# risc-mi/totalsegmentator2D

Measured on AMD Instinct MI355X. Metric: 2-ch 512x512 slices/sec, higher is better.
Workload: dtype f32 storage/accumulate, products as 3x fp16-split MFMA (f16x3)

## Files before the change

totalsegmentator2d_amd/csrc/dispatch.cpp:

```cpp
#include "engine_internal.h"
#include "tile_dims.h"

#include <algorithm>

namespace ts2d {

namespace {

inline int lg_exact(int v) { return (v > 0 && (v & (v - 1)) == 0) ? ilog2(v) : -1; }

inline void tile_finish(TileGeom& g, int B, int Ht, int Wt, int sy, int sx, int taps) {
    const bool p2 = lg_exact(g.TH) >= 0 && lg_exact(g.TW) >= 0;
    g.lgTH = p2 ? ilog2(g.TH) : -1; g.lgTW = p2 ? ilog2(g.TW) : -1;
    if (g.NIMG > 1) { g.tiles_x = 1; g.tiles_y = 1; }
    else { g.tiles_x = (Wt + g.TW - 1) / g.TW; g.tiles_y = (Ht + g.TH - 1) / g.TH; }
    g.n_mtiles = (B + g.NIMG - 1) / g.NIMG * g.tiles_x * g.tiles_y;
    const int halo = (taps == 9) ? 3 : 1;
    g.PH = (g.TH - 1) * sy + halo; g.PW = (g.TW - 1) * sx + halo;
}

TileGeom tile_geom_pow2(int B, int Ht, int Wt, int sy, int sx, int taps) {
    TileGeom g{};
    g.TW = std::min(32, pow2ceil(Wt));
    g.TH = std::min(pow2ceil(Ht), kBM / g.TW);
// ... 65 lines not shown
            if (th * tw > best || (th * tw == best && tw > g.TW)) { best = th * tw; g.TH = th; g.TW = tw; }
        }
    }
    if (best < 192) return g;
    ok = true;
    g.NIMG = 1;
    tile_finish(g, B, Ht, Wt, 2, 2, 9);
    return g;
}

TileGeom tile_fixed(int B, int Ht, int Wt, int th, int tw, int sy, int sx) {
    TileGeom g{};
    g.TH = th; g.TW = tw; g.NIMG = 1;
    tile_finish(g, B, Ht, Wt, sy, sx, 9);
    return g;
}
int choose_ksplit(const Op& op, const TileGeom& g) {
    if (op.type != OP_CONV || !op.split_ok || op.first_direct) return 1;
    if (g.NIMG < 4) return 1;
    const int nchunks = (op.cin + op.cin_skip) / (op.stride == 1 ? 16 : 8);
    int S = 1;
    while (S < 8 && nchunks / (S * 2) >= 4) S *= 2;
    return S;
}

int fill_ksplit(const ts2d_engine* e, long long n_wgs, int nchunks, bool full) {
    if (!e->use_sbk || full || e->num_cus > 256) return 1;
    int S = 1;
    while (S < 8 && n_wgs * S < e->num_cus && nchunks / (S * 2) >= 4) S *= 2;
    return S;
}

inline bool fits32(size_t bytes) { return bytes < ((size_t)1 << 31); }
inline bool magic_ok(const TileGeom& g) { return (unsigned long long)g.n_mtiles * (unsigned)(g.tiles_x * g.tiles_y) < 0x100000000ull; }

constexpr int kUpqMin = 256;
constexpr int kH2Min = 64;

int segment_tiles(const ts2d_engine* e, const TileGeom& g) {
    const int tpi = g.tiles_x * g.tiles_y, want = std::min(g.n_mtiles, 2 * e->num_cus);
    int seg = 1;
    for (int d = 1; d <= tpi; ++d) if (tpi % d == 0 && g.n_mtiles / d >= want) seg = d;
    return seg;
}

bool fuse0_applies(const ts2d_engine* e, int H, int W) {
// ... 122 lines not shown
    if (op.stride == 2) {
        int s2k = 1;
        {
            const TileGeom g1 = tile_geom(B, Ht, Wt, 2, 2, 9);
            const int P1 = g1.PH * g1.PW * g1.NIMG;
            if (e->use_one && g1.NIMG == 1 && P1 <= 5 * kBlock && img32) s2k = fill_ksplit(e, (long long)g1.n_mtiles * (op.cout / c.bn), op.cin / 8, full);
        }
        if (s2k == 1 && op.s2v2_ok && e->use_s2v2 && e->use_one && Ht % 8 == 0 && Wt % 32 == 0 && img32 && magic_ok(tile_fixed(B, Ht, Wt, 8, 32, 2, 2))) {
            c.k = K_S2_V2; c.bn = op.bn2; c.fused_stats = true;
            c.g = tile_fixed(B, Ht, Wt, 8, 32, 2, 2);
            s2v2_variant(e, op, c);
            return c;
        }
        if (s2k == 1 && op.s2v2_ok && e->use_s2v2 && e->use_one && e->use_flex2 && img32 && (f16 || e->use_flex2 > 1)) {
            bool ok = false;
            const TileGeom gs = tile_geom_s2v2(B, Ht, Wt, ok);
            if (ok && magic_ok(gs)) { c.k = K_S2_V2; c.bn = op.bn2; c.fused_stats = true; c.flex = true; c.g = gs; s2v2_variant(e, op, c); return c; }
        }
        c.g = tile_geom(B, Ht, Wt, 2, 2, 9);
        c.ksplit = std::max(choose_ksplit(op, c.g), s2k);
        c.fused_stats = c.g.NIMG == 1 && c.ksplit == 1;
        const int P = c.g.PH * c.g.PW * c.g.NIMG;
        c.k = (e->use_one && c.g.NIMG == 1 && P <= 5 * kBlock && img32) ? K_S2_ONE : K_S2_GENERIC;
        return c;
    }
    if (op.res_ok && e->use_res && e->use_one && src.normed && op.skip < 0 && Ht % 8 == 0 && Wt % 32 == 0 && fits32((size_t)Ht * Wt * 32 * 4)) {
        c.k = (oi == 1 && fuse0_applies(e, H, W)) ? K_S1_RES32F : K_S1_RES32;
        c.fused_stats = true;
        c.g = tile_fixed(B, Ht, Wt, 8, 32, 1, 1);
        c.seg = segment_tiles(e, c.g);
        return c;
    }
    c.g = tile_geom(B, Ht, Wt, 1, 1, 9);
    c.ksplit = choose_ksplit(op, c.g);
    c.fused_stats = c.g.NIMG == 1;
    const int P = c.g.PH * c.g.PW * c.g.NIMG;
    const bool srcs_normed = src.normed && (op.skip < 0 || e->tensors[op.skip].normed);
    const bool tiles16 = Ht % 16 == 0 && Wt % 32 == 0 && c.g.NIMG == 1 && img32;
    if (c.g.NIMG == 1 && img32 && op.cout % c.bn == 0) {
        const bool can = f16 ? (op.h32_ok && P * 4 <= 6 * kBlock) : (e->use_one && P * 2 <= 3 * kBlock);
        const int sk = can ? fill_ksplit(e, (long long)c.g.n_mtiles * (op.cout / c.bn), ct / (f16 ? 32 : 16), full) : 1;
        if (sk > 1) {
            c.ksplit = sk; c.fused_stats = false;
            c.k = f16 ? K_S1_H32 : K_S1_ONE;
            return c;
        }
    }
    if (f16) {
        if (e->use_h2 && tiles16 && op.cout % 64 == 0 && op.skip < 0 && ct % 32 == 0 && src.normed && ct >= kH2Min) {
            c.k = K_S1_H2; c.bn = 64;
            c.g = tile_fixed(B, Ht, Wt, 16, 32, 1, 1);
            return c;
        }
        c.k = (op.h32_ok && c.g.NIMG == 1 && P * 4 <= 6 * kBlock && img32) ? K_S1_H32 : K_S1_GENERIC;
        return c;
    }
    const bool one = e->use_one && c.g.NIMG == 1 && P * 2 <= 3 * kBlock && img32;
    if (one && e->use_q && tiles16 && c.bn == 64 && ct >= 64 && srcs_normed && magic_ok(tile_fixed(B, Ht, Wt, 16, 32, 1, 1))) {
        c.k = K_S1_QP;
        c.g = tile_fixed(B, Ht, Wt, 16, 32, 1, 1);
        return c;
    }
    c.k = one ? K_S1_ONE : K_S1_GENERIC;
    return c;
}

const char* kernel_name(const Op& op, const Choice& c) {
    const bool b64 = c.bn == 64;
    switch (c.k) {
    case K_NONE: case K_FUSED_AWAY: return "";
    case K_FIRST: return c.first_split ? "conv3x3_first_split" : "conv3x3_first";
    case K_FIRST_STATS: return "conv3x3_first_stats";
    case K_EXACT: return op.type == OP_CONV ? "conv_mfma_f32" : "convT_mfma_f32";
    case K_S1_GENERIC: return "conv3x3_f16x3";
    case K_S1_ONE: return b64 ? "conv3x3_f16x3_one<64>" : "conv3x3_f16x3_one<32>";
    case K_S1_QP: return "conv3x3_f16x3_qp";
    case K_S1_H32: return b64 ? "conv3x3_h32<64>" : "conv3x3_h32<32>";
    case K_S1_H2: return "conv3x3_h2";
    case K_S1_RES32: return "conv3x3_res32";
    case K_S1_RES32F: return "conv3x3_res32f";
    case K_S2_V2: return c.bn == 128 ? (c.k32 ? "conv3x3s2_v2<128,k32>" : "conv3x3s2_v2<128>") : (c.k32 ? "conv3x3s2_v2<64,k32>" : "conv3x3s2_v2<64>");
    case K_S2_ONE: return "conv3x3s2_f16x3_one";
    case K_S2_GENERIC: return "conv3x3s2_f16x3";
    case K_T_ONE: case K_T_GENERIC: return "convT2x2_f16x3";
    case K_UP0: return "conv3x3_up0";
    case K_UPQ: return "conv3x3_upq";
// ... 154 lines not shown
```

totalsegmentator2d_amd/csrc/engine.hip:

```cpp
#include "engine_internal.h"
#include "kernels.h"
#include "kernels_f16x3.h"
#include "kernels_f16x3_convt.h"
#include "kernels_h32.h"
#include "kernels_head.h"
#include "kernels_f16x3_one.h"
#include "kernels_f16x3_qp.h"
#include "kernels_first.h"
#include "kernels_res32.h"
#include "kernels_s2v2.h"
#include "kernels_s2v2p.h"
#include "kernels_upc.h"
#include "kernels_up0.h"
#include "kernels_upq.h"
#include "kernels_upc_h.h"
#include "kernels_upc_h2.h"
#include "kernels_resblock.h"

#include <atomic>
#include <cstdio>
#include <cmath>
#include <cstdlib>
#include <cstring>
#include <string>
// ... 339 lines not shown
    return TS2D_OK;
}

template <int TAPS, int SY, int SX, int CK, int EPI, typename ST = float>
hipError_t launch_exact_bn(bool b64, const ConvArgs& a, dim3 grid, size_t smem, hipStream_t st) {
    return b64 ? launch_max_lds<conv_mfma_f32<TAPS, SY, SX, CK, 64, EPI, ST>>(grid, dim3(kBlock), smem, st, a)
               : launch_max_lds<conv_mfma_f32<TAPS, SY, SX, CK, 32, EPI, ST>>(grid, dim3(kBlock), smem, st, a);
}
hipError_t launch_exact(int taps, int sy, int sx, int ck, int bn, bool f16, const ConvArgs& a, dim3 grid, size_t smem, hipStream_t st) {
    const bool b64 = bn == 64;
    if (bn != 32 && bn != 64) return hipErrorInvalidConfiguration;
    if (taps == 9 && sy == 1 && sx == 1 && !f16) {
        if (ck == 16) return launch_exact_bn<9, 1, 1, 16, 0>(b64, a, grid, smem, st);
        if (ck == 8) return launch_exact_bn<9, 1, 1, 8, 0>(b64, a, grid, smem, st);
    }
    if (taps == 9 && sy == 2 && sx == 2 && ck == 8 && !f16) return launch_exact_bn<9, 2, 2, 8, 0>(b64, a, grid, smem, st);
    if (taps == 9 && sy == 2 && sx == 1 && ck == 8) return f16 ? launch_exact_bn<9, 2, 1, 8, 0, _Float16>(b64, a, grid, smem, st) : launch_exact_bn<9, 2, 1, 8, 0>(b64, a, grid, smem, st);
    if (taps == 9 && sy == 1 && sx == 2 && ck == 8) return f16 ? launch_exact_bn<9, 1, 2, 8, 0, _Float16>(b64, a, grid, smem, st) : launch_exact_bn<9, 1, 2, 8, 0>(b64, a, grid, smem, st);
    if (taps == 1 && ck == 16)
        return f16 ? launch_exact_bn<1, 1, 1, 16, 1, _Float16>(b64, a, grid, smem, st) : launch_exact_bn<1, 1, 1, 16, 1>(b64, a, grid, smem, st);
    return hipErrorInvalidConfiguration;
}

hipError_t launch_tiled(Kern k, bool f16, int bn, int P, const ConvArgs& a, int grid_x, size_t smem, hipStream_t st) {
    const dim3 grid(grid_x, a.ksplit), block(kBlock);
    const bool b64 = bn == 64;
    if (bn != 32 && bn != 64) return hipErrorInvalidConfiguration;
    switch (k) {
    case K_S1_ONE:
        return b64 ? launch_max_lds<conv3x3_f16x3_one<64, true>>(grid, block, smem, st, a) : launch_max_lds<conv3x3_f16x3_one<32, false>>(grid, block, smem, st, a);
    case K_S1_H32:
        return b64 ? launch_max_lds<conv3x3_h32<64, 6>>(grid, block, smem, st, a) : launch_max_lds<conv3x3_h32<32, 6>>(grid, block, smem, st, a);
    default: break;
    }
    return with_storage(f16, [&](auto s) {
        using S = decltype(s); using ST = typename S::type;
        if (k == K_S2_ONE)
            return b64 ? launch_max_lds<conv3x3s2_f16x3_one<64, false, false, ST, S::np>>(grid, block, smem, st, a)
                       : launch_max_lds<conv3x3s2_f16x3_one<32, false, false, ST, S::np>>(grid, block, smem, st, a);
        if (k == K_S1_GENERIC) {
            if (P * 2 <= 3 * kBlock)
                return b64 ? launch_max_lds<conv3x3_f16x3<64, 3, 1, ST, S::np>>(grid, block, smem, st, a) : launch_max_lds<conv3x3_f16x3<32, 3, 1, ST, S::np>>(grid, block, smem, st, a);
            return b64 ? launch_max_lds<conv3x3_f16x3<64, 5, 1, ST, S::np>>(grid, block, smem, st, a) : launch_max_lds<conv3x3_f16x3<32, 5, 1, ST, S::np>>(grid, block, smem, st, a);
        }
        if (k == K_S2_GENERIC) {
            if (P <= 5 * kBlock)
                return b64 ? launch_max_lds<conv3x3s2_f16x3<64, 5, ST, S::np>>(grid, block, smem, st, a) : launch_max_lds<conv3x3s2_f16x3<32, 5, ST, S::np>>(grid, block, smem, st, a);
            return b64 ? launch_max_lds<conv3x3s2_f16x3<64, 6, ST, S::np>>(grid, block, smem, st, a) : launch_max_lds<conv3x3s2_f16x3<32, 6, ST, S::np>>(grid, block, smem, st, a);
        }
        return hipErrorInvalidConfiguration;
    });
}

hipError_t launch_s2v2(const ts2d_engine* e, const Choice& c, bool f16, const ConvArgs& ca, int grid_x, hipStream_t st) {
    const size_t wchunk = s2v2_wchunk(c);
    const bool resw = s2v2_resident(c);
    const dim3 grid(std::min(grid_x, 8 * ca.n_ctiles * std::max(1, e->num_cus / (8 * ca.n_ctiles)))), block(kS2Threads);
    const size_t smem = (size_t)c.npp * 2 * kS2Plane + (resw ? (size_t)c.nch : 1) * wchunk;
    if (c.s2p) return launch_max_lds<conv3x3s2_v2p>(grid, block, kS2pLds, st, ca);
    auto inst = [&](auto bn_, auto s, auto k32_) {
        using S = decltype(s); using ST = typename S::type;
        constexpr int BN = decltype(bn_)::value; constexpr bool K32 = decltype(k32_)::value;
// ... 65 lines not shown
    case K_S1_QP: {
        ca.wph = wts + op.dev_wp; ca.oscale = wts + op.dev_ws;
        const int gridp = std::min(grid, 8 * ca.n_ctiles * std::max(1, e->num_cus / (8 * ca.n_ctiles)));
        le = launch_max_lds<conv3x3_f16x3_qp>(dim3(gridp), dim3(kQThreads), kQpLds, r.st, ca);
        break;
    }
    default: {
        const bool s2 = op.stride == 2;
        size_t smem = std::max((size_t)(((P * (op.ck + 4) + 3) & ~3) + taps * (op.ck / 8) * bn * 8) * sizeof(float),
                               (size_t)4 * bn * 4 * sizeof(float));
        if (c.k != K_EXACT) {
            smem = !s2 ? (size_t)P * kRec + (size_t)9 * bn * kRec : (size_t)P * kRec8 + (size_t)5 * bn * kRec;
            smem = std::max(smem, (size_t)4 * bn * 4 * sizeof(float));
            ca.wph = wts + (c.k == K_S1_H32 ? op.dev_wh32 : op.dev_wh); ca.oscale = wts + op.dev_ws;
        }
        if (c.ksplit > 1) {
            ca.ksplit = c.ksplit; ca.kslice_stride = (long long)r.B * Ht * Wt * op.cout;
            ca.dst = e->d_partial; ca.part = nullptr;
        }
        if (smem > 160 * 1024) return fail(TS2D_ERR_INVALID, "op %s: LDS tile of %zu bytes exceeds 160 KiB", op.name.c_str(), smem);
        if (c.k == K_EXACT) {
            const bool aniso = conv ? op.stride == 3 : op.stride != 2;
            le = launch_exact(taps, conv ? op.sy : 1, conv ? op.sx : 1, op.ck, bn, r.f16 && aniso, ca, dim3(grid), smem, r.st);
        } else le = launch_tiled(c.k, r.f16, bn, P, ca, grid, smem, r.st);
        break;
    }
    }
    if (le != hipSuccess) return hip_failed(op, le);
    return TS2D_OK;
}

int launch_stats(ts2d_engine* e, size_t oi, const Choice& c, const Run& r) {
    const Op& op = e->ops[oi];
    Tensor& dst = e->tensors[op.dst];
    const float* wts = e->d_weights;
    const float *bias = wts + op.dev_b, *gamma = wts + op.dev_g, *beta = wts + op.dev_be;
    const float eps = e->arch.norm_eps;
    const int B = r.B, C = op.cout, HW = (r.H >> op.ly) * (r.W >> op.lx);
    const hipStream_t st = r.st;
    const dim3 per_image(B, C / 32);
    int ntiles = 0;
    TRY(prof_begin(e, op.name, ".stats", st)); prof_kernel(e, "finalize_stats");
    with_storage(r.f16, [&](auto s) {
        using ST = typename decltype(s)::type;
        ST* out = reinterpret_cast<ST*>(dst.data);
        const long long stride = (long long)B * HW * C;
        if (c.ksplit > 1 && HW == 256)
// ... 191 lines not shown

int ts2d_engine_weight_buffer(ts2d_engine* e, void** dev_ptr, size_t* n_bytes) {
    if (!e || !dev_ptr || !n_bytes) return fail(TS2D_ERR_INVALID, "ts2d_engine_weight_buffer: null argument");
    *dev_ptr = e->d_weights; *n_bytes = e->weight_floats * sizeof(float);
    return TS2D_OK;
}

int ts2d_engine_set_precision(ts2d_engine* e, int mode) {
    if (!e) return fail(TS2D_ERR_INVALID, "ts2d_engine_set_precision: null engine");
    if (mode != TS2D_PRECISION_F32_EXACT && mode != TS2D_PRECISION_F32_SPLIT_F16X3 && mode != TS2D_PRECISION_F16)
        return fail(TS2D_ERR_INVALID, "unknown precision mode %d", mode);
    if (mode == TS2D_PRECISION_F16 && e->residual && !e->use_resf16)
        return fail(TS2D_ERR_INVALID, "TS2D_PRECISION_F16 is not supported on a residual-encoder engine (TS2D_PRECISION_F32_SPLIT_F16X3 and "
                    "TS2D_PRECISION_F32_EXACT are); the mode is unchanged");
    e->precision = mode;
    return TS2D_OK;
}

int ts2d_engine_set_option(ts2d_engine* e, const char* name, int value) {
    if (!e || !name) return fail(TS2D_ERR_INVALID, "ts2d_engine_set_option: null argument");
    struct B { const char* n; bool* p; };
    struct I { const char* n; int* p; int lo, hi; };
    const B bools[] = {{"one", &e->use_one}, {"s2v2", &e->use_s2v2}, {"q", &e->use_q}, {"h2", &e->use_h2},  {"uh2", &e->use_uh2},
                       {"first_split", &e->use_first_split}, {"sbk", &e->use_sbk}, {"s2k32", &e->use_s2k32}, {"s2p", &e->use_s2p}, {"up0", &e->use_up0}, {"upc", &e->use_upc}, {"res", &e->use_res}, {"fuse0", &e->use_fuse0}, {"flex", &e->use_flex}, {"resf16", &e->use_resf16}};
    const I ints[] = {{"u0seg", &e->u0seg, 0, 1 << 20}, {"flex2", &e->use_flex2, 0, 2}};
    bool found = false;
    for (const B& b : bools) if (!strcmp(name, b.n)) { *b.p = value != 0; found = true; }
    for (const I& i : ints) if (!strcmp(name, i.n)) {
        if (value < i.lo || value > i.hi) return fail(TS2D_ERR_INVALID, "option %s = %d out of range [%d, %d]", name, value, i.lo, i.hi);
        *i.p = value; found = true;
    }
    if (!found) return fail(TS2D_ERR_INVALID, "unknown option '%s' (one s2v2 q h2 uh2 up0 u0seg upc res fuse0 flex flex2 first_split sbk s2k32 s2p resf16)", name);
    e->ws_precision = -1;
    ++e->opt_gen;
    return TS2D_OK;
}

int ts2d_engine_set_keep_activations(ts2d_engine* e, int enable) {
    if (!e) return fail(TS2D_ERR_INVALID, "ts2d_engine_set_keep_activations: null engine");
    e->keep_activations = enable != 0;
    return TS2D_OK;
}

int ts2d_engine_set_tile_dtype(ts2d_engine* e, int mode) {
    if (!e) return fail(TS2D_ERR_INVALID, "ts2d_engine_set_tile_dtype: null engine");
    if (mode != TS2D_TILE_F32 && mode != TS2D_TILE_F16) return fail(TS2D_ERR_INVALID, "unknown tile dtype %d", mode);
    e->tile_half = mode == TS2D_TILE_F16;
    return TS2D_OK;
}

int ts2d_engine_weights_ready(ts2d_engine* e) {
    if (!e) return fail(TS2D_ERR_INVALID, "ts2d_engine_weights_ready: null engine");
    e->weights_ready = true;
    return TS2D_OK;
}
// ... 243 lines not shown
```

totalsegmentator2d_amd/csrc/engine_internal.h:

```cpp
#pragma once
#include "../../include/ts2d_engine.h"
#include <hip/hip_runtime_api.h>
#include "device_tables.h"
#include "tile_dims.h"

#include <atomic>
#include <cstddef>
#include <cstdint>
#include <string>
#include <vector>

#pragma GCC visibility push(hidden)
namespace ts2d {

int fail(int code, const char* fmt, ...) __attribute__((format(printf, 2, 3)));
const char* last_error();

#define HIP_TRY(expr)                                                                                     \
    do {                                                                                                  \
        hipError_t _e = (expr);                                                                           \
        if (_e != hipSuccess)                                                                             \
            return fail(_e == hipErrorOutOfMemory ? TS2D_ERR_NOMEM : TS2D_ERR_HIP, "%s failed: %s (%s:%d)", \
                        #expr, hipGetErrorString(_e), __FILE__, __LINE__);                                \
    } while (0)
// ... 68 lines not shown

struct Launch { std::string name, kernel; int ksplit = 1; hipEvent_t e0 = nullptr, e1 = nullptr; };

inline size_t align_up(size_t v, size_t a) { return (v + a - 1) / a * a; }

struct TileGeom { int TH, TW, NIMG, lgTH, lgTW, tiles_x, tiles_y, n_mtiles, PH, PW; };

enum Kern { K_NONE = 0, K_FUSED_AWAY, K_FIRST, K_FIRST_STATS, K_EXACT, K_S1_GENERIC, K_S1_ONE, K_S1_QP, K_S1_H32, K_S1_H2, K_S1_RES32, K_S1_RES32F,
            K_S2_V2, K_S2_ONE, K_S2_GENERIC, K_T_ONE, K_T_GENERIC, K_UP0, K_UPQ, K_UPC, K_UPC_H, K_UPC_H2, K_HEAD_MFMA, K_HEAD_1X1, K_PROJ, K_JOIN };

struct Choice {
    Kern k = K_NONE;
    TileGeom g{};
    int bn = 0;
    int ksplit = 1;
    bool fused_stats = false;
    int ppt = 1;
    bool first_full = false;
    bool flex = false;
    bool first_split = false;
    bool k32 = false;
    int npp = 0, nch = 0;
    bool s2p = false;
    int seg = 0;
    int ks = 0;
    bool half = false;
    const char* name = "";
};

inline int pow2ceil(int v) { int p = 1; while (p < v) p <<= 1; return p; }
inline int ilog2(int v) { int l = 0; while ((1 << l) < v) ++l; return l; }
inline int ct_total(const Op& op) { return op.cin + op.cin_skip; }
inline size_t s2v2_wchunk(const Choice& c) { return (size_t)9 * c.npp * 2 * c.bn * 16; }
inline bool s2v2_resident(const Choice& c) { return (size_t)c.npp * 2 * kS2PlaneBytes + (size_t)c.nch * s2v2_wchunk(c) <= (size_t)kS2LdsMax; }

}

#pragma GCC visibility pop

struct ts2d_engine {
    ts2d_arch_desc arch{};
    int lvl_y[TS2D_MAX_STAGES] = {0}, lvl_x[TS2D_MAX_STAGES] = {0};
    int device = 0;
    int cin_pad = 8;
    std::vector<ts2d::Tensor> tensors;
    std::vector<ts2d::Op> ops;
    size_t blob_floats = 0;
    ts2d_arch_desc user_arch{};
    bool residual = false;
    int n_blocks[TS2D_MAX_STAGES] = {0};
    bool padded = false;
    size_t user_blob_floats = 0;
    float* d_weights = nullptr; size_t weight_floats = 0;
    bool weights_ready = false;
    int precision = TS2D_PRECISION_F32_SPLIT_F16X3;
    int num_cus = 256;
    int tile_half = 0;
    int tiled_inf = 0;
    bool use_one = true;
    bool use_s2v2 = true;
    bool use_q = true;
    bool use_h2 = true;
    bool use_uh2 = true;
    bool use_s2k32 = true;
    bool use_s2p = true;
    bool use_sbk = true;
    bool use_first_split = true;
    bool use_up0 = true;
    int u0seg = 0;
    bool use_upc = true;
    bool use_res = true;
    bool use_fuse0 = true;
    bool diagnosing = false;
    int use_flex2 = 2;
    bool use_resf16 = false;
    bool use_flex = true;
    int dbg = 0;
    unsigned long long* d_prof = nullptr;
    std::vector<char> fused_away;
    char* d_ws = nullptr; size_t ws_bytes = 0; int wsB = 0, wsH = 0, wsW = 0;
    bool ws_external = false;
    uint32_t ws_token = 0;
    std::vector<ts2d::Choice> plan; int planB = 0, planH = 0, planW = 0, plan_prec = -1; unsigned plan_gen = 0, opt_gen = 1; bool plan_full = false;
    char* d_stage = nullptr; size_t stage_bytes = 0;
    bool ws_full = false;
    bool last_full = false;
    int ws_precision = -1; bool ws_keep = false;
    bool keep_activations = false;
// ... 81 lines not shown
```

totalsegmentator2d_amd/csrc/kernels_f16x3.h:

```cpp
#pragma once
#include "kernels.h"

typedef _Float16 half8 __attribute__((ext_vector_type(8)));

namespace ts2d {

constexpr int kRec = 80;

template <typename ST> struct Raw8;
template <> struct Raw8<float> {
    f32x4 a, b;
    __device__ __forceinline__ void zero() { a = f32x4{0.f, 0.f, 0.f, 0.f}; b = a; }
    __device__ __forceinline__ void load(const void* base, size_t off) {
        const float* p = reinterpret_cast<const float*>(base) + off;
        a = *reinterpret_cast<const f32x4*>(p); b = *reinterpret_cast<const f32x4*>(p + 4);
    }
    __device__ __forceinline__ void get(f32x4& va, f32x4& vb) const { va = a; vb = b; }
};
template <> struct Raw8<_Float16> {
    half8 h;
    __device__ __forceinline__ void zero() {
#pragma unroll
        for (int e = 0; e < 8; ++e) h[e] = (_Float16)0.f;
    }
// ... 179 lines not shown
                const unsigned soff = (unsigned)((((rowoff & (TW - 1)) + (rowoff >> a.lgTW) * a.Wt) * a.Cout) * (int)sizeof(ST));
                float v = __builtin_fmaf(acc_t[mt][nt][i], oscale, bv);
                buffer_store_act<ST>(v, rs, voff, soff);
                const float d = round_act<ST>(v) - kv;
                s += d; q = __builtin_fmaf(d, d, q);
            }
        }
        st_s[nt] = s; st_q[nt] = q; st_k[nt] = kv;
    }
    if (a.part != nullptr) {
        lds_barrier();
        float* red = reinterpret_cast<float*>(smem8);
#pragma unroll
        for (int nt = 0; nt < NT; ++nt) {
            float s = st_s[nt], q = st_q[nt];
            s += __shfl_xor(s, 32); q += __shfl_xor(q, 32);
            if (h == 0) stat_wave_put(red, w * BN + nt * 32 + r, s, q, st_k[nt], 64.f);
        }
        lds_barrier();
        if (tid < BN) stat_tile_store(red, 4, BN, tid, a.part + ((size_t)(nimg0 * tpi + tin) * a.Cout + n0col + tid) * 4);
    }
}

template <int BN, int MAXU, int PF = 1, typename ST = float, int NP = 3>
__global__ __launch_bounds__(kBlock, 2) void conv3x3_f16x3(const ConvArgs a) {
    constexpr int NT = BN / 32;
    extern __shared__ __attribute__((aligned(16))) unsigned char smem8[];

    const int bid = blockIdx.x;
    const int xcd = bid & 7, q8 = bid >> 3;
    const int mtile = (q8 / a.n_ctiles) * 8 + xcd;
    const int ctile = q8 % a.n_ctiles;
    if (mtile >= a.n_mtiles) return;
    const int n0col = ctile * BN;

    const int NIMG = a.NIMG;
    const int tpi = a.tiles_x * a.tiles_y;
    const int grp = mtile / tpi, tin = mtile - grp * tpi;
    const int tyi = tin / a.tiles_x, txi = tin - tyi * a.tiles_x;
    const int nimg0 = grp * NIMG;
    const int ty0 = tyi * a.TH, tx0 = txi * a.TW;

    const int tid = threadIdx.x, lane = tid & 63, w = tid >> 6;
    const int r = lane & 31, h = lane >> 5;

    const int PHW = a.PH * a.PW;
    const int P = PHW * NIMG;
    unsigned char* sA = smem8;
    unsigned char* sB = smem8 + P * kRec;

    int goff[MAXU];
    unsigned long long imgbits = 0;
    const int total = P * 2;
    const float inv_phw = 1.0f / (float)PHW, inv_pw = 1.0f / (float)a.PW;
#pragma unroll
    for (int it = 0; it < MAXU; ++it) {
        const int u = tid + it * kBlock;
        int g = -1;
        if (u < total) {
            const int pp = u >> 1;
            const int il = (int)(((float)pp + 0.5f) * inv_phw), rem = pp - il * PHW;
            const int py = (int)(((float)rem + 0.5f) * inv_pw), px = rem - py * a.PW;
            const int n = nimg0 + il, iy = ty0 - 1 + py, ix = tx0 - 1 + px;
            if (n < a.B && iy >= 0 && iy < a.Hin && ix >= 0 && ix < a.Win) g = (n * a.Hin + iy) * a.Win + ix;
            imgbits |= (unsigned long long)il << (4 * it);
        }
        goff[it] = g;
    }
    const int oct = (tid & 1) * 8;

    int abase[2];
#pragma unroll
    for (int mt = 0; mt < 2; ++mt) {
        const int m = 64 * w + 32 * mt + r;
        int il, ty, tx;
        tile_row(a, m, il, ty, tx);
        abase[mt] = (il < NIMG ? (il * PHW + ty * a.PW + tx) * kRec : 0) + 16 * h;
    }
    const int bbase = r * kRec + 16 * h;

    f32x16 acc_t[2][NT];
#pragma unroll
    for (int mt = 0; mt < 2; ++mt)
#pragma unroll
        for (int nt = 0; nt < NT; ++nt)
#pragma unroll
            for (int i = 0; i < 16; ++i) acc_t[mt][nt][i] = 0.f;

    const int nchunks = (a.C0 + a.C1) / 16;
    Raw8<ST> pv[PF][MAXU];

// ... 3 lines not shown
        else { cb -= a.C0; src = a.src1; sc = a.sc1; sh = a.sh1; C = a.C1; }
    };
    auto prefetch = [&](int ch, Raw8<ST> (&pq)[MAXU]) {
        const float* src; const float* sc; const float* sh; int C, cb;
        chunk_src(ch, src, sc, sh, C, cb);
#pragma unroll
        for (int it = 0; it < MAXU; ++it) {
            pq[it].zero();
            if (goff[it] >= 0) pq[it].load(src, (size_t)goff[it] * C + cb + oct);
        }
    };

    const int kper = (nchunks + a.ksplit - 1) / a.ksplit;
    const int kbeg = (int)blockIdx.y * kper, kend = (kbeg + kper < nchunks) ? kbeg + kper : nchunks;
#pragma unroll
    for (int s = 0; s < PF; ++s) if (kbeg + s < kend) prefetch(kbeg + s, pv[s]);
    for (int ch0 = kbeg; ch0 < kend; ch0 += PF) {
#pragma unroll
    for (int s = 0; s < PF; ++s) {
        const int ch = ch0 + s;
        if (PF > 1 && ch >= kend) break;
        const float* src; const float* sc; const float* sh; int C, cb;
        chunk_src(ch, src, sc, sh, C, cb);
        __syncthreads();
        constexpr int WU = 9 * BN * 4, WIT = (WU + kBlock - 1) / kBlock;
        const uint4* wsrc = reinterpret_cast<const uint4*>(a.wph) + ((size_t)ch * a.n_ctiles + ctile) * (9 * BN * 4);
        uint4 w0, w1, w2, w3, w4, w5, w6, w7, w8;
#define TS2D_WLOAD(K, R) { const int idx = tid + K * kBlock; if (K < WIT && (WU % kBlock == 0 || idx < WU) && (NP == 3 || (idx & 2) == 0)) R = wsrc[idx]; }
        TS2D_WLOAD(0, w0) TS2D_WLOAD(1, w1) TS2D_WLOAD(2, w2) TS2D_WLOAD(3, w3) TS2D_WLOAD(4, w4)
        TS2D_WLOAD(5, w5) TS2D_WLOAD(6, w6) TS2D_WLOAD(7, w7) TS2D_WLOAD(8, w8)
#undef TS2D_WLOAD
        {
            f32x4 s1a = f32x4{1.f, 1.f, 1.f, 1.f}, s1b = s1a, s2a = f32x4{0.f, 0.f, 0.f, 0.f}, s2b = s2a;
            if (sc != nullptr && NIMG == 1 && nimg0 < a.B) {
                const size_t o = (size_t)nimg0 * C + cb + oct;
                s1a = *reinterpret_cast<const f32x4*>(sc + o); s1b = *reinterpret_cast<const f32x4*>(sc + o + 4);
                s2a = *reinterpret_cast<const f32x4*>(sh + o); s2b = *reinterpret_cast<const f32x4*>(sh + o + 4);
            }
#pragma unroll
            for (int it = 0; it < MAXU; ++it) {
                const int u = tid + it * kBlock;
                if (u < total) {
                    f32x4 va, vb;
                    pv[s][it].get(va, vb);
                    if (sc != nullptr && goff[it] >= 0) {
                        if (NIMG != 1) {
                            const size_t o = (size_t)(nimg0 + (int)((imgbits >> (4 * it)) & 15)) * C + cb + oct;
                            s1a = *reinterpret_cast<const f32x4*>(sc + o); s1b = *reinterpret_cast<const f32x4*>(sc + o + 4);
                            s2a = *reinterpret_cast<const f32x4*>(sh + o); s2b = *reinterpret_cast<const f32x4*>(sh + o + 4);
                        }
                        va = va * s1a + s2a; vb = vb * s1b + s2b;
#pragma unroll
                        for (int e = 0; e < 4; ++e) {
                            va[e] = fmaxf(va[e], va[e] * a.slope);
                            vb[e] = fmaxf(vb[e], vb[e] * a.slope);
                        }
                    }
                    half8 hi, lo;
#pragma unroll
                    for (int e = 0; e < 4; ++e) {
                        const _Float16 ha = (_Float16)va[e], hb = (_Float16)vb[e];
                        hi[e] = ha; hi[e + 4] = hb;
                        if (NP == 3) { lo[e] = (_Float16)(va[e] - (float)ha); lo[e + 4] = (_Float16)(vb[e] - (float)hb); }
                    }
                    unsigned char* d = sA + (u >> 1) * kRec + (u & 1) * 16;
                    *reinterpret_cast<half8*>(d) = hi;
                    if (NP == 3) *reinterpret_cast<half8*>(d + 32) = lo;
                }
            }
        }
#define TS2D_WSTORE(K, R) { const int idx = tid + K * kBlock; if (K < WIT && (WU % kBlock == 0 || idx < WU) && (NP == 3 || (idx & 2) == 0)) \
            *reinterpret_cast<uint4*>(sB + (idx >> 2) * kRec + (idx & 3) * 16) = R; }
        TS2D_WSTORE(0, w0) TS2D_WSTORE(1, w1) TS2D_WSTORE(2, w2) TS2D_WSTORE(3, w3) TS2D_WSTORE(4, w4)
        TS2D_WSTORE(5, w5) TS2D_WSTORE(6, w6) TS2D_WSTORE(7, w7) TS2D_WSTORE(8, w8)
#undef TS2D_WSTORE
        __syncthreads();
        if (ch + PF < kend) prefetch(ch + PF, pv[s]);

        f32x16 acc_c[2][NT];
#pragma unroll
        for (int mt = 0; mt < 2; ++mt)
#pragma unroll
            for (int nt = 0; nt < NT; ++nt)
#pragma unroll
                for (int i = 0; i < 16; ++i) acc_c[mt][nt][i] = 0.f;
        __builtin_amdgcn_s_setprio(1);
        constexpr bool PIPE = (BN == 64 && MAXU == 3);
        if constexpr (PIPE) {
        half8 fa[2][2][2], fb[2][NT][2];
        auto load_frags = [&](int buf, int tap) {
            const int toff = ((tap / 3) * a.PW + (tap % 3)) * kRec;
#pragma unroll
            for (int mt = 0; mt < 2; ++mt) {
                fa[buf][mt][0] = *reinterpret_cast<const half8*>(sA + abase[mt] + toff);
                if (NP == 3) fa[buf][mt][1] = *reinterpret_cast<const half8*>(sA + abase[mt] + toff + 32);
            }
#pragma unroll
            for (int nt = 0; nt < NT; ++nt) {
                fb[buf][nt][0] = *reinterpret_cast<const half8*>(sB + (tap * BN + nt * 32) * kRec + bbase);
                if (NP == 3) fb[buf][nt][1] = *reinterpret_cast<const half8*>(sB + (tap * BN + nt * 32) * kRec + bbase + 32);
            }
        };
        load_frags(0, 0);
#pragma unroll
        for (int tap = 0; tap < 9; ++tap) {
            const int cur = tap & 1;
            if (tap + 1 < 9) load_frags(cur ^ 1, tap + 1);
            if (NP == 3) {
#pragma unroll
                for (int mt = 0; mt < 2; ++mt)
// ... 36 lines not shown
#pragma unroll
                for (int nt = 0; nt < NT; ++nt)
                    { if (NP == 3) acc_c[mt][nt] = __builtin_amdgcn_mfma_f32_32x32x16_f16(ah[mt], bl[nt], acc_c[mt][nt], 0, 0, 0); }
#pragma unroll
            for (int mt = 0; mt < 2; ++mt)
#pragma unroll
                for (int nt = 0; nt < NT; ++nt)
                    acc_c[mt][nt] = __builtin_amdgcn_mfma_f32_32x32x16_f16(ah[mt], bh[nt], acc_c[mt][nt], 0, 0, 0);
        }
        }
        __builtin_amdgcn_s_setprio(0);
#pragma unroll
        for (int mt = 0; mt < 2; ++mt)
#pragma unroll
            for (int nt = 0; nt < NT; ++nt) acc_t[mt][nt] += acc_c[mt][nt];
    }
    }

    split_epilogue<BN, ST>(a, acc_t, smem8, n0col, nimg0, ty0, tx0, tpi, tin);
}

constexpr int kRec8 = 48;

template <int BN, int MAXU, typename ST = float, int NP = 3>
__global__ __launch_bounds__(kBlock, 2) void conv3x3s2_f16x3(const ConvArgs a) {
    constexpr int NT = BN / 32;
    extern __shared__ __attribute__((aligned(16))) unsigned char smem8[];

    const int bid = blockIdx.x;
    const int xcd = bid & 7, q8 = bid >> 3;
    const int mtile = (q8 / a.n_ctiles) * 8 + xcd;
    const int ctile = q8 % a.n_ctiles;
    if (mtile >= a.n_mtiles) return;
    const int n0col = ctile * BN;

    const int NIMG = a.NIMG;
    const int tpi = a.tiles_x * a.tiles_y;
    const int grp = mtile / tpi, tin = mtile - grp * tpi;
    const int tyi = tin / a.tiles_x, txi = tin - tyi * a.tiles_x;
    const int nimg0 = grp * NIMG;
    const int ty0 = tyi * a.TH, tx0 = txi * a.TW;

    const int tid = threadIdx.x, lane = tid & 63, w = tid >> 6;
    const int r = lane & 31, h = lane >> 5;

    const int PHW = a.PH * a.PW, PWe = (a.PW + 1) >> 1;
    const int P = PHW * NIMG;
    unsigned char* sA = smem8;
    unsigned char* sB = smem8 + P * kRec8;

    int goff[MAXU], lrec[MAXU];
    unsigned long long imgbits = 0;
    const float inv_phw = 1.0f / (float)PHW, inv_pw = 1.0f / (float)a.PW;
#pragma unroll
    for (int it = 0; it < MAXU; ++it) {
        const int u = tid + it * kBlock;
        int g = -1, lr = 0;
        if (u < P) {
            const int il = (int)(((float)u + 0.5f) * inv_phw), rem = u - il * PHW;
            const int py = (int)(((float)rem + 0.5f) * inv_pw), px = rem - py * a.PW;
            const int n = nimg0 + il, iy = 2 * ty0 - 1 + py, ix = 2 * tx0 - 1 + px;
            if (n < a.B && iy >= 0 && iy < a.Hin && ix >= 0 && ix < a.Win) g = (n * a.Hin + iy) * a.Win + ix;
            lr = (il * PHW + py * a.PW + ((px & 1) ? PWe + (px >> 1) : (px >> 1))) * kRec8;
            imgbits |= (unsigned long long)il << (4 * it);
        }
        goff[it] = g; lrec[it] = lr;
    }

    int abase[2];
#pragma unroll
    for (int mt = 0; mt < 2; ++mt) {
        const int m = 64 * w + 32 * mt + r;
        int il, ty, tx;
        tile_row(a, m, il, ty, tx);
        abase[mt] = (il < NIMG ? (il * PHW + 2 * ty * a.PW + tx) * kRec8 : 0);
    }
    int tofl[5];
#pragma unroll
    for (int s = 0; s < 5; ++s) {
        const int t = (2 * s + h) < 9 ? (2 * s + h) : 8;
        const int dy = t / 3, dx = t - 3 * dy;
        tofl[s] = (dy * a.PW + ((dx & 1) ? PWe : 0) + (dx >> 1)) * kRec8;
    }
    const int bbase = r * kRec + 16 * h;

    f32x16 acc_t[2][NT];
#pragma unroll
    for (int mt = 0; mt < 2; ++mt)
#pragma unroll
        for (int nt = 0; nt < NT; ++nt)
// ... 6 lines not shown
#pragma unroll
        for (int it = 0; it < MAXU; ++it) {
            pv[it].zero();
            if (goff[it] >= 0) pv[it].load(a.src0, (size_t)goff[it] * a.C0 + ch * 8);
        }
    };

    const int kper = (nchunks + a.ksplit - 1) / a.ksplit;
    const int kbeg = (int)blockIdx.y * kper, kend = (kbeg + kper < nchunks) ? kbeg + kper : nchunks;
    if (kbeg < kend) prefetch(kbeg);
    for (int ch = kbeg; ch < kend; ++ch) {
        const int cb = ch * 8;
        __syncthreads();
        {
            f32x4 s1a = f32x4{1.f, 1.f, 1.f, 1.f}, s1b = s1a, s2a = f32x4{0.f, 0.f, 0.f, 0.f}, s2b = s2a;
            if (a.sc0 != nullptr && NIMG == 1 && nimg0 < a.B) {
                const size_t o = (size_t)nimg0 * a.C0 + cb;
                s1a = *reinterpret_cast<const f32x4*>(a.sc0 + o); s1b = *reinterpret_cast<const f32x4*>(a.sc0 + o + 4);
                s2a = *reinterpret_cast<const f32x4*>(a.sh0 + o); s2b = *reinterpret_cast<const f32x4*>(a.sh0 + o + 4);
            }
#pragma unroll
            for (int it = 0; it < MAXU; ++it) {
                const int u = tid + it * kBlock;
                if (u < P) {
                    f32x4 va, vb;
                    pv[it].get(va, vb);
                    if (a.sc0 != nullptr && goff[it] >= 0) {
                        if (NIMG != 1) {
                            const size_t o = (size_t)(nimg0 + (int)((imgbits >> (4 * it)) & 15)) * a.C0 + cb;
                            s1a = *reinterpret_cast<const f32x4*>(a.sc0 + o); s1b = *reinterpret_cast<const f32x4*>(a.sc0 + o + 4);
                            s2a = *reinterpret_cast<const f32x4*>(a.sh0 + o); s2b = *reinterpret_cast<const f32x4*>(a.sh0 + o + 4);
                        }
                        va = va * s1a + s2a; vb = vb * s1b + s2b;
#pragma unroll
                        for (int e = 0; e < 4; ++e) {
                            va[e] = fmaxf(va[e], va[e] * a.slope);
                            vb[e] = fmaxf(vb[e], vb[e] * a.slope);
                        }
                    }
                    half8 hi, lo;
#pragma unroll
                    for (int e = 0; e < 4; ++e) {
                        const _Float16 ha = (_Float16)va[e], hb = (_Float16)vb[e];
                        hi[e] = ha; hi[e + 4] = hb;
                        if (NP == 3) { lo[e] = (_Float16)(va[e] - (float)ha); lo[e + 4] = (_Float16)(vb[e] - (float)hb); }
                    }
                    *reinterpret_cast<half8*>(sA + lrec[it]) = hi;
                    if (NP == 3) *reinterpret_cast<half8*>(sA + lrec[it] + 16) = lo;
                }
            }
        }
        {
            constexpr int WU = 5 * BN * 4;
            const uint4* wsrc = reinterpret_cast<const uint4*>(a.wph) + ((size_t)ch * a.n_ctiles + ctile) * (5 * BN * 4);
#pragma unroll
            for (int it = 0; it < (WU + kBlock - 1) / kBlock; ++it) {
                const int idx = tid + it * kBlock;
                if ((WU % kBlock == 0 || idx < WU) && (NP == 3 || (idx & 2) == 0))
                    *reinterpret_cast<uint4*>(sB + (idx >> 2) * kRec + (idx & 3) * 16) = wsrc[idx];
            }
        }
        __syncthreads();
        if (ch + 1 < kend) prefetch(ch + 1);

        f32x16 acc_c[2][NT];
#pragma unroll
        for (int mt = 0; mt < 2; ++mt)
#pragma unroll
            for (int nt = 0; nt < NT; ++nt)
#pragma unroll
                for (int i = 0; i < 16; ++i) acc_c[mt][nt][i] = 0.f;
#pragma unroll
        for (int s = 0; s < 5; ++s) {
            half8 ah[2], al[2], bh[NT], bl[NT];
#pragma unroll
            for (int mt = 0; mt < 2; ++mt) {
                ah[mt] = *reinterpret_cast<const half8*>(sA + abase[mt] + tofl[s]);
                if (NP == 3) al[mt] = *reinterpret_cast<const half8*>(sA + abase[mt] + tofl[s] + 16);
            }
#pragma unroll
            for (int nt = 0; nt < NT; ++nt) {
                bh[nt] = *reinterpret_cast<const half8*>(sB + (s * BN + nt * 32) * kRec + bbase);
                if (NP == 3) bl[nt] = *reinterpret_cast<const half8*>(sB + (s * BN + nt * 32) * kRec + bbase + 32);
            }
#pragma unroll
            for (int mt = 0; mt < 2; ++mt)
#pragma unroll
                for (int nt = 0; nt < NT; ++nt)
                    { if (NP == 3) acc_c[mt][nt] = __builtin_amdgcn_mfma_f32_32x32x16_f16(al[mt], bh[nt], acc_c[mt][nt], 0, 0, 0); }
#pragma unroll
            for (int mt = 0; mt < 2; ++mt)
#pragma unroll
                for (int nt = 0; nt < NT; ++nt)
                    { if (NP == 3) acc_c[mt][nt] = __builtin_amdgcn_mfma_f32_32x32x16_f16(ah[mt], bl[nt], acc_c[mt][nt], 0, 0, 0); }
#pragma unroll
            for (int mt = 0; mt < 2; ++mt)
#pragma unroll
                for (int nt = 0; nt < NT; ++nt)
                    acc_c[mt][nt] = __builtin_amdgcn_mfma_f32_32x32x16_f16(ah[mt], bh[nt], acc_c[mt][nt], 0, 0, 0);
        }
#pragma unroll
        for (int mt = 0; mt < 2; ++mt)
#pragma unroll
            for (int nt = 0; nt < NT; ++nt) acc_t[mt][nt] += acc_c[mt][nt];
    }
    split_epilogue<BN, ST>(a, acc_t, smem8, n0col, nimg0, ty0, tx0, tpi, tin);
}

}
```

Measured before the change: 3002.

## Add whole-image tile variants for multi-image generic conv kernels

Adds a 'whole' mode for the generic stride-1 and stride-2 f16x3 conv kernels that applies when each tile covers an entire small image (deep low-resolution layers with several images per workgroup). In this mode the kernel only loads interior pixels, zeroes the halo in LDS once, and writes through a precomputed LDS record offset, which avoids bounds checks and wasted loads on padding. It also hoists the per-image scale/shift loads ahead of the barrier for BN=64, uses a lower MAXU, and double-buffers fragment loads in the stride-2 kernel. The cost is extra template instantiations, an LDS zeroing pass, and more register pressure from the hoisted and double-buffered values.

```diff
diff --git a/totalsegmentator2d_amd/csrc/dispatch.cpp b/totalsegmentator2d_amd/csrc/dispatch.cpp
--- a/totalsegmentator2d_amd/csrc/dispatch.cpp
+++ b/totalsegmentator2d_amd/csrc/dispatch.cpp
@@ -111,6 +111,11 @@
     int S = 1;
     while (S < 8 && nchunks / (S * 2) >= 4) S *= 2;
     return S;
+}
+
+bool whole_image_tiles(const ts2d_engine* e, const TileGeom& g, int Ht, int Wt, int Hin, int Win, int stride) {
+    return e->use_whole && g.NIMG >= 2 && g.NIMG <= 16 && g.TH == Ht && g.TW == Wt && Hin == stride * Ht && Win == stride * Wt &&
+           g.NIMG * g.TH * g.TW <= kBM;
 }
 
 int fill_ksplit(const ts2d_engine* e, long long n_wgs, int nchunks, bool full) {
@@ -279,6 +284,7 @@
         c.fused_stats = c.g.NIMG == 1 && c.ksplit == 1;
         const int P = c.g.PH * c.g.PW * c.g.NIMG;
         c.k = (e->use_one && c.g.NIMG == 1 && P <= 5 * kBlock && img32) ? K_S2_ONE : K_S2_GENERIC;
+        c.whole = c.k == K_S2_GENERIC && whole_image_tiles(e, c.g, Ht, Wt, Hin, Win, 2);
         return c;
     }
     if (op.res_ok && e->use_res && e->use_one && src.normed && op.skip < 0 && Ht % 8 == 0 && Wt % 32 == 0 && fits32((size_t)Ht * Wt * 32 * 4)) {
@@ -310,6 +316,7 @@
             return c;
         }
         c.k = (op.h32_ok && c.g.NIMG == 1 && P * 4 <= 6 * kBlock && img32) ? K_S1_H32 : K_S1_GENERIC;
+        c.whole = c.k == K_S1_GENERIC && whole_image_tiles(e, c.g, Ht, Wt, Hin, Win, 1);
         return c;
     }
     const bool one = e->use_one && c.g.NIMG == 1 && P * 2 <= 3 * kBlock && img32;
@@ -319,6 +326,7 @@
         return c;
     }
     c.k = one ? K_S1_ONE : K_S1_GENERIC;
+    c.whole = c.k == K_S1_GENERIC && whole_image_tiles(e, c.g, Ht, Wt, Hin, Win, 1);
     return c;
 }
 
diff --git a/totalsegmentator2d_amd/csrc/engine.hip b/totalsegmentator2d_amd/csrc/engine.hip
--- a/totalsegmentator2d_amd/csrc/engine.hip
+++ b/totalsegmentator2d_amd/csrc/engine.hip
@@ -385,7 +385,7 @@
     return hipErrorInvalidConfiguration;
 }
 
-hipError_t launch_tiled(Kern k, bool f16, int bn, int P, const ConvArgs& a, int grid_x, size_t smem, hipStream_t st) {
+hipError_t launch_tiled(Kern k, bool f16, bool whole, int bn, int P, const ConvArgs& a, int grid_x, size_t smem, hipStream_t st) {
     const dim3 grid(grid_x, a.ksplit), block(kBlock);
     const bool b64 = bn == 64;
     if (bn != 32 && bn != 64) return hipErrorInvalidConfiguration;
@@ -401,6 +401,10 @@
         if (k == K_S2_ONE)
             return b64 ? launch_max_lds<conv3x3s2_f16x3_one<64, false, false, ST, S::np>>(grid, block, smem, st, a)
                        : launch_max_lds<conv3x3s2_f16x3_one<32, false, false, ST, S::np>>(grid, block, smem, st, a);
+        if (k == K_S1_GENERIC && whole)
+            return b64 ? launch_max_lds<conv3x3_f16x3<64, 2, 1, ST, S::np, true>>(grid, block, smem, st, a) : launch_max_lds<conv3x3_f16x3<32, 2, 1, ST, S::np, true>>(grid, block, smem, st, a);
+        if (k == K_S2_GENERIC && whole)
+            return b64 ? launch_max_lds<conv3x3s2_f16x3<64, 4, ST, S::np, true>>(grid, block, smem, st, a) : launch_max_lds<conv3x3s2_f16x3<32, 4, ST, S::np, true>>(grid, block, smem, st, a);
         if (k == K_S1_GENERIC) {
             if (P * 2 <= 3 * kBlock)
                 return b64 ? launch_max_lds<conv3x3_f16x3<64, 3, 1, ST, S::np>>(grid, block, smem, st, a) : launch_max_lds<conv3x3_f16x3<32, 3, 1, ST, S::np>>(grid, block, smem, st, a);
@@ -512,7 +516,7 @@
         if (c.k == K_EXACT) {
             const bool aniso = conv ? op.stride == 3 : op.stride != 2;
             le = launch_exact(taps, conv ? op.sy : 1, conv ? op.sx : 1, op.ck, bn, r.f16 && aniso, ca, dim3(grid), smem, r.st);
-        } else le = launch_tiled(c.k, r.f16, bn, P, ca, grid, smem, r.st);
+        } else le = launch_tiled(c.k, r.f16, c.whole, bn, P, ca, grid, smem, r.st);
         break;
     }
     }
@@ -750,7 +754,7 @@
     struct B { const char* n; bool* p; };
     struct I { const char* n; int* p; int lo, hi; };
     const B bools[] = {{"one", &e->use_one}, {"s2v2", &e->use_s2v2}, {"q", &e->use_q}, {"h2", &e->use_h2},  {"uh2", &e->use_uh2},
-                       {"first_split", &e->use_first_split}, {"sbk", &e->use_sbk}, {"s2k32", &e->use_s2k32}, {"s2p", &e->use_s2p}, {"up0", &e->use_up0}, {"upc", &e->use_upc}, {"res", &e->use_res}, {"fuse0", &e->use_fuse0}, {"flex", &e->use_flex}, {"resf16", &e->use_resf16}};
+                       {"first_split", &e->use_first_split}, {"sbk", &e->use_sbk}, {"s2k32", &e->use_s2k32}, {"s2p", &e->use_s2p}, {"whole", &e->use_whole}, {"up0", &e->use_up0}, {"upc", &e->use_upc}, {"res", &e->use_res}, {"fuse0", &e->use_fuse0}, {"flex", &e->use_flex}, {"resf16", &e->use_resf16}};
     const I ints[] = {{"u0seg", &e->u0seg, 0, 1 << 20}, {"flex2", &e->use_flex2, 0, 2}};
     bool found = false;
     for (const B& b : bools) if (!strcmp(name, b.n)) { *b.p = value != 0; found = true; }
@@ -758,7 +762,7 @@
         if (value < i.lo || value > i.hi) return fail(TS2D_ERR_INVALID, "option %s = %d out of range [%d, %d]", name, value, i.lo, i.hi);
         *i.p = value; found = true;
     }
-    if (!found) return fail(TS2D_ERR_INVALID, "unknown option '%s' (one s2v2 q h2 uh2 up0 u0seg upc res fuse0 flex flex2 first_split sbk s2k32 s2p resf16)", name);
+    if (!found) return fail(TS2D_ERR_INVALID, "unknown option '%s' (one s2v2 q h2 uh2 up0 u0seg upc res fuse0 flex flex2 first_split sbk s2k32 s2p whole resf16)", name);
     e->ws_precision = -1;
     ++e->opt_gen;
     return TS2D_OK;
diff --git a/totalsegmentator2d_amd/csrc/engine_internal.h b/totalsegmentator2d_amd/csrc/engine_internal.h
--- a/totalsegmentator2d_amd/csrc/engine_internal.h
+++ b/totalsegmentator2d_amd/csrc/engine_internal.h
@@ -114,6 +114,7 @@
     bool k32 = false;
     int npp = 0, nch = 0;
     bool s2p = false;
+    bool whole = false;
     int seg = 0;
     int ks = 0;
     bool half = false;
@@ -156,6 +157,7 @@
     bool use_uh2 = true;
     bool use_s2k32 = true;
     bool use_s2p = true;
+    bool use_whole = true;
     bool use_sbk = true;
     bool use_first_split = true;
     bool use_up0 = true;
diff --git a/totalsegmentator2d_amd/csrc/kernels_f16x3.h b/totalsegmentator2d_amd/csrc/kernels_f16x3.h
--- a/totalsegmentator2d_amd/csrc/kernels_f16x3.h
+++ b/totalsegmentator2d_amd/csrc/kernels_f16x3.h
@@ -225,7 +225,11 @@
     }
 }
 
-template <int BN, int MAXU, int PF = 1, typename ST = float, int NP = 3>
+__device__ __forceinline__ void zero_patch(unsigned char* sA, int bytes) {
+    for (int i = threadIdx.x * 16; i < bytes; i += kBlock * 16) *reinterpret_cast<uint4*>(sA + i) = uint4{0u, 0u, 0u, 0u};
+}
+
+template <int BN, int MAXU, int PF = 1, typename ST = float, int NP = 3, bool WHOLE = false>
 __global__ __launch_bounds__(kBlock, 2) void conv3x3_f16x3(const ConvArgs a) {
     constexpr int NT = BN / 32;
     extern __shared__ __attribute__((aligned(16))) unsigned char smem8[];
@@ -252,24 +256,35 @@
     unsigned char* sA = smem8;
     unsigned char* sB = smem8 + P * kRec;
 
-    int goff[MAXU];
+    int goff[MAXU], lrec[WHOLE ? MAXU : 1];
     unsigned long long imgbits = 0;
-    const int total = P * 2;
-    const float inv_phw = 1.0f / (float)PHW, inv_pw = 1.0f / (float)a.PW;
+    const int total = WHOLE ? NIMG * a.TH * a.TW * 2 : P * 2;
+    const float inv_phw = 1.0f / (float)(WHOLE ? a.TH * a.TW : PHW), inv_pw = 1.0f / (float)(WHOLE ? a.TW : a.PW);
 #pragma unroll
     for (int it = 0; it < MAXU; ++it) {
         const int u = tid + it * kBlock;
         int g = -1;
         if (u < total) {
             const int pp = u >> 1;
-            const int il = (int)(((float)pp + 0.5f) * inv_phw), rem = pp - il * PHW;
-            const int py = (int)(((float)rem + 0.5f) * inv_pw), px = rem - py * a.PW;
-            const int n = nimg0 + il, iy = ty0 - 1 + py, ix = tx0 - 1 + px;
-            if (n < a.B && iy >= 0 && iy < a.Hin && ix >= 0 && ix < a.Win) g = (n * a.Hin + iy) * a.Win + ix;
-            imgbits |= (unsigned long long)il << (4 * it);
-        }
+            if constexpr (WHOLE) {
+                const int thw = a.TH * a.TW;
+                const int il = (int)(((float)pp + 0.5f) * inv_phw), rem = pp - il * thw;
+                const int y = (int)(((float)rem + 0.5f) * inv_pw), x = rem - y * a.TW;
+                const int n = nimg0 + il;
+                if (n < a.B) g = (n * a.Hin + y) * a.Win + x;
+                lrec[it] = (il * PHW + (y + 1) * a.PW + x + 1) * kRec + (u & 1) * 16;
+                imgbits |= (unsigned long long)il << (4 * it);
+            } else {
+                const int il = (int)(((float)pp + 0.5f) * inv_phw), rem = pp - il * PHW;
+                const int py = (int)(((float)rem + 0.5f) * inv_pw), px = rem - py * a.PW;
+                const int n = nimg0 + il, iy = ty0 - 1 + py, ix = tx0 - 1 + px;
+                if (n < a.B && iy >= 0 && iy < a.Hin && ix >= 0 && ix < a.Win) g = (n * a.Hin + iy) * a.Win + ix;
+                imgbits |= (unsigned long long)il << (4 * it);
+            }
+        } else if constexpr (WHOLE) lrec[it] = 0;
         goff[it] = g;
     }
+    if constexpr (WHOLE) zero_patch(sA, P * kRec);
     const int oct = (tid & 1) * 8;
 
     int abase[2];
@@ -319,6 +334,17 @@
         if (PF > 1 && ch >= kend) break;
         const float* src; const float* sc; const float* sh; int C, cb;
         chunk_src(ch, src, sc, sh, C, cb);
+        constexpr bool HOIST = WHOLE && BN == 64;
+        f32x4 q1a[HOIST ? MAXU : 1], q1b[HOIST ? MAXU : 1], q2a[HOIST ? MAXU : 1], q2b[HOIST ? MAXU : 1];
+        if constexpr (HOIST) {
+#pragma unroll
+            for (int it = 0; it < MAXU; ++it)
+                if (sc != nullptr && goff[it] >= 0) {
+                    const size_t o = (size_t)(nimg0 + (int)((imgbits >> (4 * it)) & 15)) * C + cb + oct;
+                    q1a[it] = *reinterpret_cast<const f32x4*>(sc + o); q1b[it] = *reinterpret_cast<const f32x4*>(sc + o + 4);
+                    q2a[it] = *reinterpret_cast<const f32x4*>(sh + o); q2b[it] = *reinterpret_cast<const f32x4*>(sh + o + 4);
+                }
+        }
         __syncthreads();
         constexpr int WU = 9 * BN * 4, WIT = (WU + kBlock - 1) / kBlock;
         const uint4* wsrc = reinterpret_cast<const uint4*>(a.wph) + ((size_t)ch * a.n_ctiles + ctile) * (9 * BN * 4);
@@ -337,11 +363,12 @@
 #pragma unroll
             for (int it = 0; it < MAXU; ++it) {
                 const int u = tid + it * kBlock;
-                if (u < total) {
+                if (WHOLE ? goff[it] >= 0 : u < total) {
                     f32x4 va, vb;
                     pv[s][it].get(va, vb);
                     if (sc != nullptr && goff[it] >= 0) {
-                        if (NIMG != 1) {
+                        if constexpr (HOIST) { s1a = q1a[it]; s1b = q1b[it]; s2a = q2a[it]; s2b = q2b[it]; }
+                        else if (NIMG != 1) {
                             const size_t o = (size_t)(nimg0 + (int)((imgbits >> (4 * it)) & 15)) * C + cb + oct;
                             s1a = *reinterpret_cast<const f32x4*>(sc + o); s1b = *reinterpret_cast<const f32x4*>(sc + o + 4);
                             s2a = *reinterpret_cast<const f32x4*>(sh + o); s2b = *reinterpret_cast<const f32x4*>(sh + o + 4);
@@ -353,16 +380,24 @@
                             vb[e] = fmaxf(vb[e], vb[e] * a.slope);
                         }
                     }
-                    half8 hi, lo;
-#pragma unroll
-                    for (int e = 0; e < 4; ++e) {
-                        const _Float16 ha = (_Float16)va[e], hb = (_Float16)vb[e];
-                        hi[e] = ha; hi[e + 4] = hb;
-                        if (NP == 3) { lo[e] = (_Float16)(va[e] - (float)ha); lo[e + 4] = (_Float16)(vb[e] - (float)hb); }
+                    if constexpr (WHOLE && NP == 3) {
+                        uint4 hi, lo;
+                        split_hi_lo_8(va, vb, hi, lo);
+                        *reinterpret_cast<uint4*>(sA + lrec[it]) = hi;
+                        *reinterpret_cast<uint4*>(sA + lrec[it] + 32) = lo;
+                    } else {
+                        half8 hi, lo;
+#pragma unroll
+                        for (int e = 0; e < 4; ++e) {
+                            const _Float16 ha = (_Float16)va[e], hb = (_Float16)vb[e];
+                            hi[e] = ha; hi[e + 4] = hb;
+                            if (NP == 3) { lo[e] = (_Float16)(va[e] - (float)ha); lo[e + 4] = (_Float16)(vb[e] - (float)hb); }
+                        }
+                        unsigned char* d = sA + (u >> 1) * kRec + (u & 1) * 16;
+                        if constexpr (WHOLE) d = sA + lrec[it];
+                        *reinterpret_cast<half8*>(d) = hi;
+                        if (NP == 3) *reinterpret_cast<half8*>(d + 32) = lo;
                     }
-                    unsigned char* d = sA + (u >> 1) * kRec + (u & 1) * 16;
-                    *reinterpret_cast<half8*>(d) = hi;
-                    if (NP == 3) *reinterpret_cast<half8*>(d + 32) = lo;
                 }
             }
         }
@@ -382,7 +417,7 @@
 #pragma unroll
                 for (int i = 0; i < 16; ++i) acc_c[mt][nt][i] = 0.f;
         __builtin_amdgcn_s_setprio(1);
-        constexpr bool PIPE = (BN == 64 && MAXU == 3);
+        constexpr bool PIPE = (BN == 64 && MAXU <= 3);
         if constexpr (PIPE) {
         half8 fa[2][2][2], fb[2][NT][2];
         auto load_frags = [&](int buf, int tap) {
@@ -465,7 +500,7 @@
 
 constexpr int kRec8 = 48;
 
-template <int BN, int MAXU, typename ST = float, int NP = 3>
+template <int BN, int MAXU, typename ST = float, int NP = 3, bool WHOLE = false>
 __global__ __launch_bounds__(kBlock, 2) void conv3x3s2_f16x3(const ConvArgs a) {
     constexpr int NT = BN / 32;
     extern __shared__ __attribute__((aligned(16))) unsigned char smem8[];
@@ -494,12 +529,21 @@
 
     int goff[MAXU], lrec[MAXU];
     unsigned long long imgbits = 0;
-    const float inv_phw = 1.0f / (float)PHW, inv_pw = 1.0f / (float)a.PW;
+    const float inv_phw = 1.0f / (float)(WHOLE ? a.Hin * a.Win : PHW), inv_pw = 1.0f / (float)(WHOLE ? a.Win : a.PW);
 #pragma unroll
     for (int it = 0; it < MAXU; ++it) {
         const int u = tid + it * kBlock;
         int g = -1, lr = 0;
-        if (u < P) {
+        if constexpr (WHOLE) {
+            if (u < NIMG * a.Hin * a.Win) {
+                const int il = (int)(((float)u + 0.5f) * inv_phw), rem = u - il * (a.Hin * a.Win);
+                const int y = (int)(((float)rem + 0.5f) * inv_pw), x = rem - y * a.Win;
+                const int n = nimg0 + il, px = x + 1;
+                if (n < a.B) g = (n * a.Hin + y) * a.Win + x;
+                lr = (il * PHW + (y + 1) * a.PW + ((px & 1) ? PWe + (px >> 1) : (px >> 1))) * kRec8;
+                imgbits |= (unsigned long long)il << (4 * it);
+            }
+        } else if (u < P) {
             const int il = (int)(((float)u + 0.5f) * inv_phw), rem = u - il * PHW;
             const int py = (int)(((float)rem + 0.5f) * inv_pw), px = rem - py * a.PW;
             const int n = nimg0 + il, iy = 2 * ty0 - 1 + py, ix = 2 * tx0 - 1 + px;
@@ -509,6 +553,7 @@
         }
         goff[it] = g; lrec[it] = lr;
     }
+    if constexpr (WHOLE) zero_patch(sA, P * kRec8);
 
     int abase[2];
 #pragma unroll
@@ -561,7 +606,7 @@
 #pragma unroll
             for (int it = 0; it < MAXU; ++it) {
                 const int u = tid + it * kBlock;
-                if (u < P) {
+                if (WHOLE ? goff[it] >= 0 : u < P) {
                     f32x4 va, vb;
                     pv[it].get(va, vb);
                     if (a.sc0 != nullptr && goff[it] >= 0) {
@@ -577,15 +622,22 @@
                             vb[e] = fmaxf(vb[e], vb[e] * a.slope);
                         }
                     }
-                    half8 hi, lo;
-#pragma unroll
-                    for (int e = 0; e < 4; ++e) {
-                        const _Float16 ha = (_Float16)va[e], hb = (_Float16)vb[e];
-                        hi[e] = ha; hi[e + 4] = hb;
-                        if (NP == 3) { lo[e] = (_Float16)(va[e] - (float)ha); lo[e + 4] = (_Float16)(vb[e] - (float)hb); }
+                    if constexpr (WHOLE && NP == 3) {
+                        uint4 hi, lo;
+                        split_hi_lo_8(va, vb, hi, lo);
+                        *reinterpret_cast<uint4*>(sA + lrec[it]) = hi;
+                        *reinterpret_cast<uint4*>(sA + lrec[it] + 16) = lo;
+                    } else {
+                        half8 hi, lo;
+#pragma unroll
+                        for (int e = 0; e < 4; ++e) {
+                            const _Float16 ha = (_Float16)va[e], hb = (_Float16)vb[e];
+                            hi[e] = ha; hi[e + 4] = hb;
+                            if (NP == 3) { lo[e] = (_Float16)(va[e] - (float)ha); lo[e + 4] = (_Float16)(vb[e] - (float)hb); }
+                        }
+                        *reinterpret_cast<half8*>(sA + lrec[it]) = hi;
+                        if (NP == 3) *reinterpret_cast<half8*>(sA + lrec[it] + 16) = lo;
                     }
-                    *reinterpret_cast<half8*>(sA + lrec[it]) = hi;
-                    if (NP == 3) *reinterpret_cast<half8*>(sA + lrec[it] + 16) = lo;
                 }
             }
         }
@@ -609,34 +661,42 @@
             for (int nt = 0; nt < NT; ++nt)
 #pragma unroll
                 for (int i = 0; i < 16; ++i) acc_c[mt][nt][i] = 0.f;
+        constexpr bool AHEAD = WHOLE;
+        half8 ah[AHEAD ? 2 : 1][2], al[AHEAD ? 2 : 1][2], bh[AHEAD ? 2 : 1][NT], bl[AHEAD ? 2 : 1][NT];
+        auto load_frags = [&](int buf, int s) {
+#pragma unroll
+            for (int mt = 0; mt < 2; ++mt) {
+                ah[buf][mt] = *reinterpret_cast<const half8*>(sA + abase[mt] + tofl[s]);
+                if (NP == 3) al[buf][mt] = *reinterpret_cast<const half8*>(sA + abase[mt] + tofl[s] + 16);
+            }
+#pragma unroll
+            for (int nt = 0; nt < NT; ++nt) {
+                bh[buf][nt] = *reinterpret_cast<const half8*>(sB + (s * BN + nt * 32) * kRec + bbase);
+                if (NP == 3) bl[buf][nt] = *reinterpret_cast<const half8*>(sB + (s * BN + nt * 32) * kRec + bbase + 32);
+            }
+        };
+        if (AHEAD) load_frags(0, 0);
 #pragma unroll
         for (int s = 0; s < 5; ++s) {
-            half8 ah[2], al[2], bh[NT], bl[NT];
-#pragma unroll
-            for (int mt = 0; mt < 2; ++mt) {
-                ah[mt] = *reinterpret_cast<const half8*>(sA + abase[mt] + tofl[s]);
-                if (NP == 3) al[mt] = *reinterpret_cast<const half8*>(sA + abase[mt] + tofl[s] + 16);
-            }
-#pragma unroll
-            for (int nt = 0; nt < NT; ++nt) {
-                bh[nt] = *reinterpret_cast<const half8*>(sB + (s * BN + nt * 32) * kRec + bbase);
-                if (NP == 3) bl[nt] = *reinterpret_cast<const half8*>(sB + (s * BN + nt * 32) * kRec + bbase + 32);
-            }
+            const int cur = AHEAD ? (s & 1) : 0;
+            if (!AHEAD) load_frags(0, s);
+            else if (s + 1 < 5) load_frags(cur ^ 1, s + 1);
 #pragma unroll
             for (int mt = 0; mt < 2; ++mt)
 #pragma unroll
                 for (int nt = 0; nt < NT; ++nt)
-                    { if (NP == 3) acc_c[mt][nt] = __builtin_amdgcn_mfma_f32_32x32x16_f16(al[mt], bh[nt], acc_c[mt][nt], 0, 0, 0); }
+                    { if (NP == 3) acc_c[mt][nt] = __builtin_amdgcn_mfma_f32_32x32x16_f16(al[cur][mt], bh[cur][nt], acc_c[mt][nt], 0, 0, 0); }
 #pragma unroll
             for (int mt = 0; mt < 2; ++mt)
 #pragma unroll
                 for (int nt = 0; nt < NT; ++nt)
-                    { if (NP == 3) acc_c[mt][nt] = __builtin_amdgcn_mfma_f32_32x32x16_f16(ah[mt], bl[nt], acc_c[mt][nt], 0, 0, 0); }
+                    { if (NP == 3) acc_c[mt][nt] = __builtin_amdgcn_mfma_f32_32x32x16_f16(ah[cur][mt], bl[cur][nt], acc_c[mt][nt], 0, 0, 0); }
 #pragma unroll
             for (int mt = 0; mt < 2; ++mt)
 #pragma unroll
                 for (int nt = 0; nt < NT; ++nt)
-                    acc_c[mt][nt] = __builtin_amdgcn_mfma_f32_32x32x16_f16(ah[mt], bh[nt], acc_c[mt][nt], 0, 0, 0);
+                    acc_c[mt][nt] = __builtin_amdgcn_mfma_f32_32x32x16_f16(ah[cur][mt], bh[cur][nt], acc_c[mt][nt], 0, 0, 0);
+            if (AHEAD) __builtin_amdgcn_sched_barrier(0);
         }
 #pragma unroll
         for (int mt = 0; mt < 2; ++mt)
```

After: 3016 (median of 6 runs). No clear change (+0.5%).
